# javieryu/nn_distributed_training

Measured on NVIDIA H100. Metric: consensus node-rounds/sec (DiNNO, dist_mnist_PAPER; rounds/sec x graph nodes), higher is better.
Workload: dtype fp64

## Files before the change

### nn_distributed_training_b200/ops/csrc/mnist_cl64.cu

```cuda
#include "mnist_device.cuh"

namespace nndt {
namespace mnist {

namespace cl64 {

constexpr int NT = 512, CL = 4, CELLS = 36, KC = 108, WS = 116, HS = 68;
constexpr int PXR = 10 * HW;
constexpr int KT = (KC + 7) / 8;
constexpr int HR = 68;
NNDT_DEVINL int hr(int j) { return (j >> 4) * 17 + (j & 15); }
constexpr int PART_WC = 0, PART_BC = 75, PART_B1 = 78, PART_W2 = 142, PART_B2 = 782, PART_LOSS = 792, PART_N = 793;

template <int MS>
struct Smem {
  static constexpr int NO = MS / CL;
  static constexpr bool kDoublePix = MS <= 32;
  static constexpr int PXS = kDoublePix ? PXR + 2 : PXR;
  double w[HID * WS];
  double a[MS * WS];
  double h[MS * HS];
  alignas(16) unsigned char img[kDoublePix ? MS * PXS * 8 : MS * PXS];
  double lut[kDoublePix ? 1 : 256];
  double h_loc[NO * HR > CL * 80 ? NO * HR : CL * 80];
  double dh_loc[NO * HID];
  double part[800];
  double w2[NCLS * HR];
  alignas(16) double b1[HID];
  alignas(16) double b2[16];
  double wc[80];
  double dz[NO * 16];
  double red[NO];
  int sidx[MS];
  int label[MS];
  float valid[MS];
  unsigned char arg[MS * KC];
};
static_assert(sizeof(Smem<16>) <= 227 * 1024 && sizeof(Smem<32>) <= 227 * 1024 && sizeof(Smem<64>) <= 227 * 1024,
              "shared memory budget");

NNDT_DEVINL double wmax(double v) {
#pragma unroll
  for (int o = 16; o > 0; o >>= 1) v = fmax(v, __shfl_xor_sync(0xffffffffu, v, o));
  return v;
}
template <int H>
NNDT_DEVINL void fold_half(double (&v)[16], int lane) {
  const bool up = (lane & (2 * H)) != 0;
#pragma unroll
  for (int i = 0; i < H; ++i) {
    const double send = up ? v[i] : v[i + H], keep = up ? v[i + H] : v[i];
    v[i] = keep + __shfl_xor_sync(0xffffffffu, send, 2 * H);
  }
}
NNDT_DEVINL void warp_reduce_scatter16(double (&v)[16], int lane) {
  fold_half<8>(v, lane); fold_half<4>(v, lane); fold_half<2>(v, lane); fold_half<1>(v, lane);
  v[0] += __shfl_xor_sync(0xffffffffu, v[0], 1);
}
NNDT_DEVINL void dmma_nv(double (&c)[4], double a0, double a1, double b) {
  asm("mma.sync.aligned.m16n8k4.row.col.f64.f64.f64.f64 {%0,%1,%2,%3}, {%4,%5}, {%6}, {%0,%1,%2,%3};"
      : "+d"(c[0]), "+d"(c[1]), "+d"(c[2]), "+d"(c[3])
      : "d"(a0), "d"(a1), "d"(b));
}
template <int NJ, int K, class FA, class FB>
NNDT_DEVINL void gemm_k(double (&c)[NJ][4], int m0, int n0, int lane, FA A, FB B) {
  static_assert(K % 4 == 0, "k steps of 4");
  const int g = lane >> 2, t = lane & 3;
  double a0 = A(m0 + g, t), a1 = A(m0 + g + 8, t), b[NJ];
#pragma unroll
  for (int j = 0; j < NJ; ++j) b[j] = B(t, n0 + 8 * j + g);
#pragma unroll
  for (int k0 = 0; k0 < K; k0 += 4) {
    double na0 = 0.0, na1 = 0.0, nb[NJ];
    if (k0 + 4 < K) {
      const int k = k0 + 4 + t;
      na0 = A(m0 + g, k); na1 = A(m0 + g + 8, k);
#pragma unroll
      for (int j = 0; j < NJ; ++j) nb[j] = B(k, n0 + 8 * j + g);
    }
#pragma unroll
    for (int j = 0; j < NJ; ++j) dmma_nv(c[j], a0, a1, b[j]);
    if (k0 + 4 < K) {
      a0 = na0; a1 = na1;
#pragma unroll
      for (int j = 0; j < NJ; ++j) b[j] = nb[j];
    }
  }
}
NNDT_DEVINL void stamp(long long* prof, int idx, int tid) {
  if (prof != nullptr && tid == 0) {
    long long t;
    asm volatile("mov.u64 %0, %%globaltimer;" : "=l"(t));
    prof[idx] = t;
  }
}

template <int MS>
__global__ void __cluster_dims__(CL, 1, 1) __launch_bounds__(NT, 1)
mnist_cl64_train_kernel(const Args a, const GenericShape gs) {
  using SM = Smem<MS>;
  constexpr int NO = SM::NO, PXS = SM::PXS;
  constexpr bool kDoublePix = SM::kDoublePix;
  static_assert(MS % 16 == 0 && NO <= NT / 32, "tile geometry");
  static_assert(CELLS % 2 == 0 && NCLS % 2 == 0 && 32 + NCLS / 2 <= NT, "16-byte parameter copies");
  extern __shared__ __align__(16) unsigned char smem_raw[];
  SM& sm = *reinterpret_cast<SM*>(smem_raw);
  const int tid = threadIdx.x, warp = tid >> 5, lane = tid & 31;
  const int l = blockIdx.z, bsplit = blockIdx.y, nsplit = gridDim.y;
  const int c = (int)cluster_rank();
  const double* th = reinterpret_cast<const double*>(a.theta) + (size_t)l * a.n_pad;
  const double pmean = gs.mean, pis = gs.inv_std;
  const bool u8 = a.x_is_u8 != 0;
  double* imgd = reinterpret_cast<double*>(sm.img);
  auto pix = [&](int s, int p) -> double {
    if constexpr (kDoublePix) return imgd[s * PXS + p];
    else if (u8) return sm.lut[sm.img[s * PXR + p]];
    else return (double)__ldg(reinterpret_cast<const float*>(a.x) + (size_t)sm.sidx[s] * 784 + 6 * HW * c + p);
  };
  long long* prof = a.prof != nullptr ? a.prof + ((l * nsplit + bsplit) * CL + c) * 64 : nullptr;
  stamp(prof, 0, tid);

  const int call = a.calls != nullptr ? a.calls[l] : 0;
  const BatchGeom bg = batch_geom<true>(a, l, call);
  if (tid < MS) {
    int idx = 0, lab = 0; float ok = 0.f;
    const uint32_t t = (uint32_t)(bsplit * MS + tid);
    if (t < bg.bs) {
      ok = 1.f;
      idx = a.direct ? (int)(l * a.batch + t) : bg.shard_off + (int)feistel_permute(bg.start + t, bg.m, bg.key);
      lab = (int)a.y[idx];
    }
    sm.sidx[tid] = idx; sm.valid[tid] = ok; sm.label[tid] = lab;
  }
  if constexpr (!kDoublePix)
    if (tid < 256) sm.lut[tid] = ((double)tid * (1.0 / 255.0) - pmean) * pis;
  __syncthreads();
  constexpr int NU8 = (MS * 35 + NT - 1) / NT, NF4 = kDoublePix ? (MS * 70 + NT - 1) / NT : 1;
  uint2 pu[NU8]; float4 pf[NF4];
  if (u8) {
#pragma unroll
    for (int i = 0; i < NU8; ++i) {
      const int o = tid + i * NT;
      pu[i] = make_uint2(0, 0);
      if (o < MS * 35) {
        const int s = o / 35, q = o - s * 35;
        if (sm.valid[s] != 0.f)
          pu[i] = *reinterpret_cast<const uint2*>(reinterpret_cast<const unsigned char*>(a.x) + (size_t)sm.sidx[s] * 784 + 6 * HW * c + 8 * q);
      }
    }
  } else if constexpr (kDoublePix) {
#pragma unroll
    for (int i = 0; i < NF4; ++i) {
      const int o = tid + i * NT;
      pf[i] = make_float4(0.f, 0.f, 0.f, 0.f);
      if (o < MS * 70) {
        const int s = o / 70, q = o - s * 70;
        if (sm.valid[s] != 0.f)
          pf[i] = *reinterpret_cast<const float4*>(reinterpret_cast<const float*>(a.x) + (size_t)sm.sidx[s] * 784 + 6 * HW * c + 4 * q);
      }
    }
  }
  if (u8) {
#pragma unroll
    for (int i = 0; i < NU8; ++i) {
      const int o = tid + i * NT;
      if (o < MS * 35) {
        const int s = o / 35, q = o - s * 35;
        if constexpr (kDoublePix) {
          const uint32_t w[2] = {pu[i].x, pu[i].y};
          double* dst = imgd + s * PXS + 8 * q;
#pragma unroll
          for (int j = 0; j < 8; ++j) dst[j] = ((double)((w[j >> 2] >> (8 * (j & 3))) & 0xff) * (1.0 / 255.0) - pmean) * pis;
        } else {
          *reinterpret_cast<uint2*>(sm.img + s * PXR + 8 * q) = pu[i];
        }
      }
    }
  } else if constexpr (kDoublePix) {
#pragma unroll
    for (int i = 0; i < NF4; ++i) {
      const int o = tid + i * NT;
      if (o < MS * 70) {
        double* dst = imgd + (o / 70) * PXS + 4 * (o % 70);
        dst[0] = pf[i].x; dst[1] = pf[i].y; dst[2] = pf[i].z; dst[3] = pf[i].w;
      }
    }
  }
  stamp(prof, 1, tid);
  pdl_wait();
  pdl_launch_dependents();
  stamp(prof, 2, tid);

  constexpr int NW2 = (NCLS * HID + NT - 1) / NT;
  double wcv = 0.0, w2v[NW2];
  if (tid < 75) wcv = __ldcg(th + a.off_wc + tid);
  else if (tid < 78) wcv = __ldcg(th + a.off_bc + (tid - 75));
#pragma unroll
  for (int i = 0; i < NW2; ++i) {
    const int o = tid + i * NT;
    w2v[i] = o < NCLS * HID ? __ldcg(th + a.off_w2 + o) : 0.0;
  }
  for (int o = tid; o < HID * KC / 2; o += NT) {
    const int j = o / (KC / 2), r = o - j * (KC / 2), ch = r / (CELLS / 2), q = 2 * (r - ch * (CELLS / 2));
    cp_async16(sm.w + j * WS + ch * CELLS + q, th + a.off_w1 + (size_t)j * FC1_IN + ch * NPOOL + CELLS * c + q);
  }
  if (tid < HID / 2) cp_async16(sm.b1 + 2 * tid, th + a.off_b1 + 2 * tid);
  else if (tid >= 32 && tid < 32 + NCLS / 2) cp_async16(sm.b2 + 2 * (tid - 32), th + a.off_b2 + 2 * (tid - 32));
  cp_async_commit();
  if (tid < 78) sm.wc[tid] = wcv;
#pragma unroll
  for (int i = 0; i < NW2; ++i) {
    const int o = tid + i * NT;
    if (o < NCLS * HID) sm.w2[(o / HID) * HR + hr(o % HID)] = w2v[i];
  }
  __syncthreads();
  stamp(prof, 3, tid);

  for (int it = tid; it < MS * CELLS; it += NT) {
    const int s = it / CELLS, cell = it - s * CELLS;
    const int pr = cell / PHW, px = cell - pr * PHW;
    const int p0 = (2 * pr) * HW + 2 * px;
    double patch[6][6];
    if constexpr (kDoublePix) {
      const double* src = imgd + s * PXS + p0;
#pragma unroll
      for (int r = 0; r < 6; ++r)
#pragma unroll
        for (int q = 0; q < 6; q += 2) {
          const double2 v = *reinterpret_cast<const double2*>(src + r * HW + q);
          patch[r][q] = v.x; patch[r][q + 1] = v.y;
        }
    } else {
#pragma unroll
      for (int r = 0; r < 6; ++r)
#pragma unroll
        for (int q = 0; q < 6; ++q) patch[r][q] = pix(s, p0 + r * HW + q);
    }
    const bool ok = sm.valid[s] != 0.f;
#pragma unroll 1
    for (int ch = 0; ch < F; ++ch) {
      double a00 = 0, a01 = 0, a10 = 0, a11 = 0;
#pragma unroll
      for (int ky = 0; ky < KS; ++ky)
#pragma unroll
        for (int kx = 0; kx < KS; ++kx) {
          const double w = sm.wc[ch * 25 + ky * 5 + kx];
          a00 += w * patch[ky][kx]; a01 += w * patch[ky][kx + 1];
          a10 += w * patch[ky + 1][kx]; a11 += w * patch[ky + 1][kx + 1];
        }
      double m = a00; int ai = 0;
      if (a01 > m) { m = a01; ai = 1; }
      if (a10 > m) { m = a10; ai = 2; }
      if (a11 > m) { m = a11; ai = 3; }
      m += sm.wc[75 + ch];
      m = (ok && m > 0.0) ? m : 0.0;
      sm.a[s * WS + ch * CELLS + cell] = m;
      sm.arg[s * KC + ch * CELLS + cell] = (unsigned char)(ai | (m > 0.0 ? 4 : 0));
    }
  }
  cp_async_wait<0>();
  __syncthreads();
  stamp(prof, 4, tid);

  {
    constexpr int NJ1 = MS == 64 ? 2 : 1, NGRP = 8 / NJ1;
    if (warp < (MS / 16) * NGRP) {
      const int m0 = 16 * (warp / NGRP), n0 = 8 * NJ1 * (warp % NGRP);
      double acc[NJ1][4];
      zero(acc);
      gemm_k<NJ1, KC>(acc, m0, n0, lane, at(sm.a, WS), at_t(sm.w, WS));
#pragma unroll
      for (int j = 0; j < NJ1; ++j)
#pragma unroll
        for (int i = 0; i < 4; ++i) sm.h[frow(m0, lane, i) * HS + fcol(n0 + 8 * j, lane, i)] = acc[j][i];
    }
  }
  stamp(prof, 5, tid);
  cluster_sync();
  stamp(prof, 6, tid);
  if (c == 0 && tid == 0 && a.calls != nullptr) {
    if (a.arrive == nullptr || nsplit == 1) a.calls[l] = call + 1;
    else if (atomicAdd(a.arrive + l, 1u) == (unsigned)nsplit - 1) { a.arrive[l] = 0; a.calls[l] = call + 1; }
  }

  const int s0 = c * NO;
  const double inv_bs = 1.0 / (double)(bg.bs ? bg.bs : 1);
  if (warp < NO) {
    const int sl = warp, s = s0 + sl;
    double hv[2];
#pragma unroll
    for (int q = 0; q < 2; ++q) {
      const int j = lane + 32 * q;
      const double* src = sm.h + s * HS + j;
      double v = sm.b1[j];
#pragma unroll
      for (int r = 0; r < CL; ++r) v += ld_dsmem(map_to(src, (uint32_t)r));
      hv[q] = v > 0.0 ? v : 0.0;
      sm.h_loc[sl * HR + hr(j)] = hv[q];
    }
    __syncwarp();
    double zp[2];
#pragma unroll
    for (int r = 0; r < 2; ++r) {
      const int o = lane + 32 * r, cc = o >> 2, part = o & 3;
      double v = 0.0;
      if (o < 4 * NCLS) {
#pragma unroll
        for (int jj = 0; jj < 16; ++jj) v += sm.h_loc[sl * HR + part * 17 + jj] * sm.w2[cc * HR + part * 17 + jj];
      }
      v += __shfl_xor_sync(0xffffffffu, v, 1);
      v += __shfl_xor_sync(0xffffffffu, v, 2);
      zp[r] = v;
    }
    static_assert(NCLS > 8 && NCLS <= 16, "two rounds of four lanes per class");
    const double z0 = __shfl_sync(0xffffffffu, zp[0], (4 * lane) & 31), z1 = __shfl_sync(0xffffffffu, zp[1], (4 * lane) & 31);
    const bool cls = lane < NCLS;
    const double zc = cls ? (lane < 8 ? z0 : z1) + sm.b2[lane] : -1.0e300;
    const double mx = wmax(zc);
    const double se = warp_sum(cls ? exp(zc - mx) : 0.0);
    const double lse = mx + log(se);
    const int y = sm.label[s];
    const double ok = (double)sm.valid[s];
    const double dzc = cls ? ok * inv_bs * (exp(zc - lse) - (lane == y ? 1.0 : 0.0)) : 0.0;
    if (cls) sm.dz[sl * 16 + lane] = dzc;
    if (lane == y) sm.red[sl] = ok * (lse - zc);
    double dh[2] = {0.0, 0.0};
#pragma unroll
    for (int cc = 0; cc < NCLS; ++cc) {
      const double d = __shfl_sync(0xffffffffu, dzc, cc);
      dh[0] += d * sm.w2[cc * HR + hr(lane)];
      dh[1] += d * sm.w2[cc * HR + hr(lane + 32)];
    }
#pragma unroll
    for (int q = 0; q < 2; ++q) sm.dh_loc[sl * HID + lane + 32 * q] = hv[q] > 0.0 ? dh[q] : 0.0;
  }
  __syncthreads();
  for (int o = tid; o < NCLS * HID; o += NT) {
    const int cc = o >> 6, j = o & 63;
    double v = 0.0;
    for (int sl = 0; sl < NO; ++sl) v += sm.dz[sl * 16 + cc] * sm.h_loc[sl * HR + hr(j)];
    sm.part[PART_W2 + o] = v;
  }
  if (tid < HID) {
    double v = 0.0;
    for (int sl = 0; sl < NO; ++sl) v += sm.dh_loc[sl * HID + tid];
    sm.part[PART_B1 + tid] = v;
  } else if (tid >= 64 && tid < 64 + NCLS) {
    double v = 0.0;
    for (int sl = 0; sl < NO; ++sl) v += sm.dz[sl * 16 + (tid - 64)];
    sm.part[PART_B2 + (tid - 64)] = v;
  } else if (tid == 96) {
    double v = 0.0;
    for (int sl = 0; sl < NO; ++sl) v += sm.red[sl];
    sm.part[PART_LOSS] = v * inv_bs;
  }
  stamp(prof, 7, tid);
  cluster_sync();
  stamp(prof, 8, tid);
  double* gp = reinterpret_cast<double*>(a.grad_part) + ((size_t)l * nsplit + bsplit) * a.n_pad;
  {
    constexpr int NE = PART_N - PART_B1, PER = (NE + CL - 1) / CL;
    const int o = PART_B1 + c * PER + tid;
    if (tid < PER && o < PART_N) {
      double v = 0.0;
#pragma unroll
      for (int r = 0; r < CL; ++r) v += ld_dsmem(map_to(sm.part + o, (uint32_t)r));
      if (o < PART_W2) gp[a.off_b1 + (o - PART_B1)] = v;
      else if (o < PART_B2) gp[a.off_w2 + (o - PART_W2)] = v;
      else if (o < PART_LOSS) gp[a.off_b2 + (o - PART_B2)] = v;
      else {
        a.loss_part[l * nsplit + bsplit] = (float)v;
        if (a.loss_mirror != nullptr) a.loss_mirror[l * nsplit + bsplit] = (float)v;
      }
    }
  }
  for (int o = tid; o < MS * HID; o += NT) {
    const int s = o >> 6, j = o & 63, r = s / NO;
    sm.h[s * HS + j] = ld_dsmem(map_to(sm.dh_loc + (s - r * NO) * HID + j, (uint32_t)r));
  }
  __syncthreads();
  stamp(prof, 9, tid);

  constexpr int NP2 = (MS / 16) * (KT / 2), NR2 = (NP2 + NT / 32 - 1) / (NT / 32);
  static_assert(KT % 2 == 0 && KC * MS + (NT / 32) * 16 <= HID * WS, "da1 and the conv-grad warp sums fit in the W slice");
  double acc2[NR2][2][4];
#pragma unroll
  for (int r = 0; r < NR2; ++r) {
    zero(acc2[r]);
    const int p = warp + r * (NT / 32);
    if (p < NP2) gemm_k<2, HID>(acc2[r], 16 * (p / (KT / 2)), 16 * (p % (KT / 2)), lane, at(sm.h, HS), at(sm.w, WS));
  }
  __syncthreads();
  stamp(prof, 10, tid);
  double* da1 = sm.w;
#pragma unroll
  for (int r = 0; r < NR2; ++r) {
    const int p = warp + r * (NT / 32);
    if (p < NP2) {
      const int m0 = 16 * (p / (KT / 2)), n0 = 16 * (p % (KT / 2));
#pragma unroll
      for (int jt = 0; jt < 2; ++jt)
#pragma unroll
        for (int i = 0; i < 4; ++i) {
          const int s = frow(m0, lane, i), k = fcol(n0 + 8 * jt, lane, i);
          if (k < KC) da1[k * MS + s] = (sm.arg[s * KC + k] & 4) ? acc2[r][jt][i] : 0.0;
        }
    }
  }
  __syncthreads();
  stamp(prof, 11, tid);
  constexpr int W3 = NT / 32 - HID / 16, NJ3 = KT / 2;
  if (warp >= W3) {
    const int m0 = 16 * (warp - W3);
#pragma unroll 1
    for (int n0 = 0; n0 < 8 * KT; n0 += 8 * NJ3) {
      double acc[NJ3][4];
      zero(acc);
      gemm_k<NJ3, MS>(acc, m0, n0, lane, at_t(sm.h, HS), at(sm.a, WS));
#pragma unroll
      for (int jt = 0; jt < NJ3; ++jt)
#pragma unroll
        for (int i = 0; i < 4; i += 2) {
          const int j = frow(m0, lane, i), k = fcol(n0 + 8 * jt, lane, i);
          if (k < KC) {
            const int ch = k / CELLS, cell = k - ch * CELLS;
            __stcg(reinterpret_cast<double2*>(gp + a.off_w1 + (size_t)j * FC1_IN + ch * NPOOL + CELLS * c + cell),
                   make_double2(acc[jt][i], acc[jt][i + 1]));
          }
        }
    }
    stamp(prof, 12, tid - W3 * 32);
  }
  constexpr int KW = 3, NRUN = MS * 3;
  static_assert(KS * KW < NT / 32 && F * KS <= 16, "conv-grad work split");
  double* wsums = sm.w + KC * MS;
  auto pix2 = [&](int s, int p) -> double2 {
    if constexpr (kDoublePix) return *reinterpret_cast<const double2*>(imgd + s * PXS + p);
    else return make_double2(pix(s, p), pix(s, p + 1));
  };
  if (warp < KS * KW) {
    const int ky = warp / KW;
    double acc[16];
#pragma unroll
    for (int i = 0; i < 16; ++i) acc[i] = 0.0;
#pragma unroll 1
    for (int r = tid - ky * KW * 32; r < NRUN; r += KW * 32) {
      const int s = r % MS, pr = r / MS;
      const int rb = (2 * pr + ky) * HW;
      double x0[6], x1[6];
#pragma unroll
      for (int px = 0; px < PHW; ++px) {
        const int p = rb + 2 * px;
        if (px == 0) {
#pragma unroll
          for (int q = 0; q < 6; q += 2) {
            const double2 u = pix2(s, p + q), v = pix2(s, p + HW + q);
            x0[q] = u.x; x0[q + 1] = u.y; x1[q] = v.x; x1[q + 1] = v.y;
          }
        } else {
#pragma unroll
          for (int q = 0; q < 4; ++q) { x0[q] = x0[q + 2]; x1[q] = x1[q + 2]; }
          const double2 u = pix2(s, p + 4), v = pix2(s, p + HW + 4);
          x0[4] = u.x; x0[5] = u.y; x1[4] = v.x; x1[5] = v.y;
        }
#pragma unroll
        for (int ch = 0; ch < F; ++ch) {
          const int k = ch * CELLS + pr * PHW + px;
          const double g = da1[k * MS + s];
          const int ai = sm.arg[s * KC + k] & 3;
          const double g00 = ai == 0 ? g : 0.0, g01 = ai == 1 ? g : 0.0, g10 = ai == 2 ? g : 0.0, g11 = ai == 3 ? g : 0.0;
#pragma unroll
          for (int kx = 0; kx < KS; ++kx) {
            double& t = acc[ch * KS + kx];
            t = fma(g00, x0[kx], t); t = fma(g01, x0[kx + 1], t);
            t = fma(g10, x1[kx], t); t = fma(g11, x1[kx + 1], t);
          }
        }
      }
    }
    warp_reduce_scatter16(acc, lane);
    if ((lane & 1) == 0 && (lane >> 1) < F * KS) wsums[warp * 16 + (lane >> 1)] = acc[0];
  } else if (warp == KS * KW) {
#pragma unroll 1
    for (int ch = 0; ch < F; ++ch) {
      double v = 0.0;
      for (int o = lane; o < CELLS * MS; o += 32) v += da1[ch * CELLS * MS + o];
      v = warp_sum(v);
      if (lane == 0) wsums[warp * 16 + ch] = v;
    }
  }
  __syncthreads();
  if (tid < 78) {
    double v = 0.0;
    if (tid < 75) {
      const int ch = tid / 25, t = tid - ch * 25, ky = t / KS, kx = t - ky * KS;
#pragma unroll
      for (int w = 0; w < KW; ++w) v += wsums[(ky * KW + w) * 16 + ch * KS + kx];
    } else {
      v = wsums[KS * KW * 16 + (tid - 75)];
    }
    st_dsmem(map_to(sm.h_loc + c * 80 + tid, 0u), v);
  }
  stamp(prof, 13, tid);
  cluster_sync();
  if (c == 0 && tid < 78) {
    double v = 0.0;
#pragma unroll
    for (int r = 0; r < CL; ++r) v += sm.h_loc[r * 80 + tid];
    gp[tid < 75 ? a.off_wc + tid : a.off_bc + (tid - 75)] = v;
  }
  stamp(prof, 14, tid);
}

template <int MS>
static cudaError_t prepare_ms() {
  static cudaError_t prep = cudaFuncSetAttribute(mnist_cl64_train_kernel<MS>, cudaFuncAttributeMaxDynamicSharedMemorySize, (int)sizeof(Smem<MS>));
  return prep;
}

template <int MS>
static cudaError_t launch_ms(const Args& a, const GenericShape& gs, cudaStream_t st) {
  const cudaError_t prep = prepare_ms<MS>();
  if (prep != cudaSuccess) return prep;
  cudaLaunchConfig_t cfg{};
  cfg.gridDim = dim3(CL, 64 / MS, a.L); cfg.blockDim = dim3(NT);
  cfg.dynamicSmemBytes = sizeof(Smem<MS>); cfg.stream = st;
  cudaLaunchAttribute attr[1];
  attr[0].id = cudaLaunchAttributeProgrammaticStreamSerialization;
  attr[0].val.programmaticStreamSerializationAllowed = 1;
  static const bool no_pdl = getenv("NNDT_NO_PDL") != nullptr;
  cfg.attrs = attr; cfg.numAttrs = no_pdl ? 0 : 1;
  return cudaLaunchKernelEx(&cfg, mnist_cl64_train_kernel<MS>, a, gs);
}

template <int MS>
static int max_clusters_ms() {
  if (prepare_ms<MS>() != cudaSuccess) { cudaGetLastError(); return 0; }
  cudaLaunchConfig_t cfg{};
  cfg.gridDim = dim3(CL, 1, 1); cfg.blockDim = dim3(NT); cfg.dynamicSmemBytes = sizeof(Smem<MS>);
  int n = 0;
  if (cudaOccupancyMaxActiveClusters(&n, mnist_cl64_train_kernel<MS>, &cfg) != cudaSuccess) { cudaGetLastError(); return 0; }
  return n;
}

}

cudaError_t launch_train_cl64(const Args& a, const GenericShape& gs, int nsplit, cudaStream_t st) {
  switch (nsplit) {
    case 1: return cl64::launch_ms<64>(a, gs, st);
    case 2: return cl64::launch_ms<32>(a, gs, st);
    case 4: return cl64::launch_ms<16>(a, gs, st);
  }
  return cudaErrorInvalidValue;
}

int cl64_max_active_clusters(int nsplit) {
  switch (nsplit) {
    case 1: return cl64::max_clusters_ms<64>();
    case 2: return cl64::max_clusters_ms<32>();
    case 4: return cl64::max_clusters_ms<16>();
  }
  return 0;
}

int cl64_cluster_ctas() { return cl64::CL; }

}
}
```

Measured before the change: 161,100.

## Spread fc1 weight-grad GEMM across all warps and halve conv-grad FMAs

The fc1 weight-gradient DMMA GEMM previously ran on the last four warps only, each looping over all column tiles. It is now split across all 16 warps, one 16-row block per SM sub-partition, with 4/4/3/3 tile groups. The first 8 warps run it before the conv-gradient phase and the rest after it, to balance those phases. The conv-gradient inner loop now selects the pooled-argmax row once and does two FMAs per tap instead of four, at the cost of per-element selects into a temporary array.

```diff
diff --git a/nn_distributed_training_b200/ops/csrc/mnist_cl64.cu b/nn_distributed_training_b200/ops/csrc/mnist_cl64.cu
--- a/nn_distributed_training_b200/ops/csrc/mnist_cl64.cu
+++ b/nn_distributed_training_b200/ops/csrc/mnist_cl64.cu
@@ -87,6 +87,22 @@
     }
   }
 }
+template <int NJ, int MS>
+NNDT_DEVINL void dw1_tiles(const double* dh, const double* at_, double* gw, int m0, int n0, int lane) {
+  double acc[NJ][4];
+  zero(acc);
+  gemm_k<NJ, MS>(acc, m0, n0, lane, at_t(dh, HS), at(at_, WS));
+#pragma unroll
+  for (int jt = 0; jt < NJ; ++jt)
+#pragma unroll
+    for (int i = 0; i < 4; i += 2) {
+      const int j = frow(m0, lane, i), k = fcol(n0 + 8 * jt, lane, i);
+      if (k < KC) {
+        const int ch = k / CELLS, cell = k - ch * CELLS;
+        __stcg(reinterpret_cast<double2*>(gw + (size_t)j * FC1_IN + ch * NPOOL + cell), make_double2(acc[jt][i], acc[jt][i + 1]));
+      }
+    }
+}
 NNDT_DEVINL void stamp(long long* prof, int idx, int tid) {
   if (prof != nullptr && tid == 0) {
     long long t;
@@ -409,27 +425,17 @@
   }
   __syncthreads();
   stamp(prof, 11, tid);
-  constexpr int W3 = NT / 32 - HID / 16, NJ3 = KT / 2;
-  if (warp >= W3) {
-    const int m0 = 16 * (warp - W3);
-#pragma unroll 1
-    for (int n0 = 0; n0 < 8 * KT; n0 += 8 * NJ3) {
-      double acc[NJ3][4];
-      zero(acc);
-      gemm_k<NJ3, MS>(acc, m0, n0, lane, at_t(sm.h, HS), at(sm.a, WS));
-#pragma unroll
-      for (int jt = 0; jt < NJ3; ++jt)
-#pragma unroll
-        for (int i = 0; i < 4; i += 2) {
-          const int j = frow(m0, lane, i), k = fcol(n0 + 8 * jt, lane, i);
-          if (k < KC) {
-            const int ch = k / CELLS, cell = k - ch * CELLS;
-            __stcg(reinterpret_cast<double2*>(gp + a.off_w1 + (size_t)j * FC1_IN + ch * NPOOL + CELLS * c + cell),
-                   make_double2(acc[jt][i], acc[jt][i + 1]));
-          }
-        }
-    }
-    stamp(prof, 12, tid - W3 * 32);
+  static_assert(HID / 16 == 4 && KT == 14, "GEMM 3 split: one 16-row block per SM sub-partition, 4 + 4 + 3 + 3 tiles");
+  auto gemm3 = [&]() {
+    const int q = warp & 3, i = warp >> 2, m0 = 16 * q, n0 = 8 * (4 * i - (i > 2 ? i - 2 : 0));
+    double* gw = gp + a.off_w1 + CELLS * c;
+    if (i < 2) dw1_tiles<4, MS>(sm.h, sm.a, gw, m0, n0, lane);
+    else dw1_tiles<3, MS>(sm.h, sm.a, gw, m0, n0, lane);
+  };
+  const bool g3_first = warp < 8;
+  if (g3_first) {
+    gemm3();
+    stamp(prof, 12, tid);
   }
   constexpr int KW = 3, NRUN = MS * 3;
   static_assert(KS * KW < NT / 32 && F * KS <= 16, "conv-grad work split");
@@ -468,12 +474,15 @@
           const int k = ch * CELLS + pr * PHW + px;
           const double g = da1[k * MS + s];
           const int ai = sm.arg[s * KC + k] & 3;
-          const double g00 = ai == 0 ? g : 0.0, g01 = ai == 1 ? g : 0.0, g10 = ai == 2 ? g : 0.0, g11 = ai == 3 ? g : 0.0;
+          const bool dy = (ai & 2) != 0, dx = (ai & 1) != 0;
+          const double g0 = dx ? 0.0 : g, g1 = dx ? g : 0.0;
+          double xr[6];
+#pragma unroll
+          for (int q = 0; q < 6; ++q) xr[q] = dy ? x1[q] : x0[q];
 #pragma unroll
           for (int kx = 0; kx < KS; ++kx) {
             double& t = acc[ch * KS + kx];
-            t = fma(g00, x0[kx], t); t = fma(g01, x0[kx + 1], t);
-            t = fma(g10, x1[kx], t); t = fma(g11, x1[kx + 1], t);
+            t = fma(g0, xr[kx], t); t = fma(g1, xr[kx + 1], t);
           }
         }
       }
@@ -489,6 +498,7 @@
       if (lane == 0) wsums[warp * 16 + ch] = v;
     }
   }
+  if (!g3_first) gemm3();
   __syncthreads();
   if (tid < 78) {
     double v = 0.0;
```

Measured after the change: 161,800, median of 6. Within noise of the previous version (+0.5%).
